# sony/timbre-trap

Measured on AMD Instinct MI355X. Metric: audio-seconds/s training throughput (9oct x 60bpo, 3s@22.05kHz), higher is better.
Workload: dtype bf16; 1 GPU; full train step (CQT x2 + AE fwd/bwd with consistency + 3 losses + clip + AdamW), model_complexity=2 latent=128, 64 clips x 3 s per GPU, under torch.autocast like reference experiments/train.py:415 (bf16 MFMA conv path of BASELINE config[2]; fp32 master weights, losses and optimizer); global_batch=64, parallelism=dp1

## Files before the change

include/ttrap.h:

```cpp
#ifndef TTRAP_H
#define TTRAP_H

#include <stdint.h>

#ifdef __cplusplus
extern "C" {
#endif

#define TT_E_BADARG      (-1)
#define TT_W_JOIN_LEFT 1
#define TT_E_UNSUPPORTED (-2)

#define TT_FLAG_BF16_OPERANDS 1
#define TT_FLAG_BF16_SPLIT    2

#define TT_ACT_NONE 0
#define TT_ACT_ELU  1
#define TT_ACT_RELU    2
#define TT_ACT_SIGMOID 3

int         tt_version(void);
const char* tt_arch(void);
const char* tt_error_string(int code);
int         tt_set_cu_limit(int cus);
// ... 124 lines not shown

int64_t tt_latent16_scratch_bytes(int B, int CT, int D, int E, int T);
int tt_latent16_contract(const void* in, const void* gy, const float* w, const float* bias, float* out, void* ws, int B, int CT,
                         int D, int Dout, int E, int T, void* stream);
int tt_latent16_expand(const float* z, int Dz, float fill, const float* w, const float* bias, void* out, void* ws, int B, int CT,
                       int D, int E, int T, void* stream);
int tt_latent16_pregated_ok(int CT, int D);
int tt_latent16_expand_gated(const float* z, const float* w, const void* gy, void* out, void* ws, int B, int CT, int D, int E, int T,
                             void* stream);
int tt_latent16_contract_pregated(const void* g, const float* w, float* out, void* ws, int B, int CT, int D, int Dout, int E, int T,
                                  void* stream);
int tt_latent16_wgrad_pregated(const float* z, int Dz, float fill, const void* g, float* dw, float* db, void* ws, int B, int CT, int D,
                               int E, int T, void* stream);
int tt_latent16_wgrad(const float* z, int Dz, float fill, const void* g, const void* gy, float* dw, float* db, void* ws, int B,
                      int CT, int D, int E, int T, void* stream);

int64_t tt_edge16_scratch_bytes(void);
int tt_convin16_fwd(const float* x, const float* w, const float* b, void* y, int B, int H, int T, void* stream);
int tt_convin16_bwd(const float* x, const void* y, const void* dy, const float* w, float* dx, float* dw, float* db, void* ws,
                    int B, int H, int T, void* stream);
int tt_convout16_fwd(const void* x, const float* w, const float* b, float* y, int B, int H, int T, void* stream);
int tt_convout16_bwd(const void* x, const float* dy, const float* w, void* dx, float* dw, float* db, void* ws, int B, int H,
                     int T, void* stream);
int tt_convin16_1_fwd(const float* x, const float* w, const float* b, void* y, int B, int H, int T, void* stream);
int tt_convin16_1_bwd(const float* x, const void* y, const void* dy, const float* w, float* dx, float* dw, float* db, void* ws, int B,
                      int H, int T, void* stream);
int tt_convout16_1_fwd(const void* x, const float* w, const float* b, float* y, int B, int H, int T, int act, void* stream);
int tt_convout16_1_bwd(const void* x, const float* y, const float* dy, const float* w, void* dx, float* dw, float* db, void* ws, int B,
                       int H, int T, int act, void* stream);

// ... 232 lines not shown
```

timbre-trap_amd/csrc/latent_bf16.hip:

```cpp
#include "bf16_common.h"

namespace {

#ifndef LAT_WGRAD_WAVES
#define LAT_WGRAD_WAVES 4
#endif
#ifndef LAT_EXPAND_Q
#define LAT_EXPAND_Q 2
#endif
#ifndef LAT_NSPLIT
#define LAT_NSPLIT 32
#endif

__device__ __forceinline__ float gate_f(float dy, float y) { return dy * elu_dout(y); }

template <int CT> __device__ __forceinline__ int ochc(int ct, int m) { return (CT / 4) * (m >> 2) + 4 * ct + (m & 3); }

template <int CT, int DT>
__global__ __launch_bounds__(NT) void k_lat_wprep1(const float* __restrict__ w, e16* __restrict__ wp, int D, int E) {
    constexpr int SPH = CT / 32;
    const int i = blockIdx.x * NT + threadIdx.x;
    if (i >= E * SPH * DT * 64) return;
    const int lane = i & 63, dt = (i >> 6) % DT, s = (i >> 6) / DT;
    const int h = s / SPH, half = s - h * SPH;
// ... 19 lines not shown
__global__ __launch_bounds__(NT) void k_lat_zprep(const float* __restrict__ z, e16* __restrict__ zt, int D, int Dz, float fill, int T,
                                                   long npix, float zscale, int one_row = -1) {
    constexpr int ZS = 32 * KS + 16, PCS = ZS / 8;
    const long i = (long)blockIdx.x * NT + threadIdx.x;
    const long pix = (i / (64 * PCS)) * 64 + (i & 63);
    if (pix >= npix) return;
    const int d0 = (int)((i >> 6) % PCS) * 8;
    const long b = pix / T, t = pix - b * T;
    e16x8 v;
#pragma unroll
    for (int e = 0; e < 8; ++e)
        v[e] = (e16)(zscale * (d0 + e < Dz ? z[(b * Dz + d0 + e) * T + t] : (d0 + e < D ? fill : (d0 + e == one_row ? 1.f : 0.f))));
    *reinterpret_cast<e16x8*>(zt + pix * ZS + d0) = v;
}

template <int CT, int DT, bool GATE, int QN>
__global__ __launch_bounds__(NT) void k_lat_contract(const e16* __restrict__ in, const e16* __restrict__ gy,
                                                      const e16* __restrict__ wp, const float* __restrict__ bias,
                                                      float* __restrict__ out, int D, int Dout, int E, int T, long npix, float oscale) {
    constexpr int SPH = CT / 32;
    constexpr int CHUNK = DT * 64 * 16, ROUNDS = (DT * 64 + NT - 1) / NT;
    extern __shared__ __align__(16) unsigned char smem[];
    const int tid = threadIdx.x, lane = tid & 63, wave = tid >> 6;
    const int n = lane & 15, g = lane >> 4;
    const int nsteps = E * SPH;
    const long p0 = (long)blockIdx.x * (64 * QN) + wave * (16 * QN);
    long pix[QN]; bool ok[QN]; long base[QN];
#pragma unroll
    for (int q = 0; q < QN; ++q) {
        pix[q] = p0 + 16 * q + n;
        ok[q] = pix[q] < npix;
        const long b = pix[q] / T, t = pix[q] - b * T;
        base[q] = (b * E * T + t) * CT + 8 * g;
    }
    auto stage = [&](int s, int buf) {
        const e16* src = wp + (long)s * (DT * 64 * 8);
#pragma unroll
        for (int r = 0; r < ROUNDS; ++r) {
            const int i = r * NT + wave * 64, p = i + lane;
            glds16(src + (long)(p < DT * 64 ? p : DT * 64 - 1) * 8, smem + buf * (ROUNDS * NT * 16) + (long)i * 16);
        }
    };
    auto fetch = [&](int s, e16x8 (&q8)[QN]) {
        const int h = s / SPH, half = s - h * SPH;
#pragma unroll
        for (int q = 0; q < QN; ++q) {
            const long off = base[q] + (long)h * T * CT + 32 * half;
            const bool live = ok[q] && s < nsteps;
            e16x8 v = *reinterpret_cast<const e16x8*>(in + (live ? off : 0));
            if (GATE) {
                const e16x8 yv = *reinterpret_cast<const e16x8*>(gy + (live ? off : 0));
#pragma unroll
                for (int e = 0; e < 8; ++e) v[e] = (e16)gate_f((float)v[e], (float)yv[e]);
            }
            if (!live)
#pragma unroll
                for (int e = 0; e < 8; ++e) v[e] = (e16)0.f;
            q8[q] = v;
        }
    };
    f32x4 acc[DT][QN];
#pragma unroll
    for (int dt = 0; dt < DT; ++dt)
#pragma unroll
        for (int q = 0; q < QN; ++q) acc[dt][q] = f32x4{0.f, 0.f, 0.f, 0.f};
    e16x8 bq[QN], bn[QN];
    stage(0, 0);
    fetch(0, bq);
    for (int s = 0; s < nsteps; ++s) {
        asm volatile("s_waitcnt vmcnt(0)" ::: "memory");
        __syncthreads();
        if (s + 1 < nsteps) stage(s + 1, (s + 1) & 1);
        fetch(s + 1, bn);
        const unsigned char* wb = smem + (s & 1) * (ROUNDS * NT * 16);
#pragma unroll
        for (int dt = 0; dt < DT; ++dt) {
            const e16x8 a = *reinterpret_cast<const e16x8*>(wb + ((long)dt * 64 + lane) * 16);
#pragma unroll
            for (int q = 0; q < QN; ++q) acc[dt][q] = mma32(a, bq[q], acc[dt][q]);
        }
#pragma unroll
        for (int q = 0; q < QN; ++q) bq[q] = bn[q];
    }
#pragma unroll
    for (int q = 0; q < QN; ++q) {
        if (!ok[q]) continue;
        const long b = pix[q] / T, t = pix[q] - b * T;
#pragma unroll
        for (int dt = 0; dt < DT; ++dt)
#pragma unroll
            for (int r = 0; r < 4; ++r) {
                const int d = 16 * dt + 4 * g + r;
                if (d < Dout) out[(b * Dout + d) * T + t] = acc[dt][q][r] * oscale + (bias ? bias[d] : 0.f);
            }
    }
    (void)CHUNK;
}

template <int CT, int KS, bool ACT, int QE, bool GOUT = false>
__global__ __launch_bounds__(NT) void k_lat_expand(const e16* __restrict__ zt, const e16* __restrict__ wp,
                                                    const float* __restrict__ bias, e16* __restrict__ out, int E, int T,
                                                    long npix, const e16* __restrict__ gy = nullptr) {
    constexpr int NC = CT / 16, NCH = CT / 4, ZS = 32 * KS + 16;
    constexpr int PCS = NC * KS * 64, ROUNDS = (PCS + NT - 1) / NT;
    extern __shared__ __align__(16) unsigned char smem[];
    const int tid = threadIdx.x, lane = tid & 63, wave = tid >> 6;
    const int n = lane & 15, g = lane >> 4;
    const long p0 = (long)blockIdx.x * (64 * QE) + wave * (16 * QE);
    e16x8 bz[QE][KS];
    long obase[QE]; bool ok[QE];
#pragma unroll
    for (int q = 0; q < QE; ++q) {
        const long pix = p0 + 16 * q + n;
        ok[q] = pix < npix;
        const long pc = ok[q] ? pix : 0;
#pragma unroll
        for (int s = 0; s < KS; ++s) bz[q][s] = *reinterpret_cast<const e16x8*>(zt + pc * ZS + 32 * s + 8 * g);
        const long b = pc / T, t = pc - b * T;
        obase[q] = (b * E * T + t) * CT + NCH * g;
    }
    float br[NCH];
#pragma unroll
    for (int e = 0; e < NCH; ++e) br[e] = ACT ? bias[NCH * g + e] : 0.f;
    auto stage = [&](int h, int buf) {
        const e16* src = wp + (long)h * (PCS * 8);
#pragma unroll
        for (int r = 0; r < ROUNDS; ++r) {
            const int i = r * NT + wave * 64, p = i + lane;
            glds16(src + (long)(p < PCS ? p : PCS - 1) * 8, smem + buf * (ROUNDS * NT * 16) + (long)i * 16);
        }
    };
    stage(0, 0);
    for (int h = 0; h < E; ++h) {
        asm volatile("s_waitcnt vmcnt(0)" ::: "memory");
        __syncthreads();
        if (h + 1 < E) stage(h + 1, (h + 1) & 1);
        const unsigned char* wb = smem + (h & 1) * (ROUNDS * NT * 16);
        f32x4 acc[NC][QE];
#pragma unroll
        for (int ct = 0; ct < NC; ++ct)
#pragma unroll
            for (int q = 0; q < QE; ++q) acc[ct][q] = f32x4{0.f, 0.f, 0.f, 0.f};
#pragma unroll
        for (int ct = 0; ct < NC; ++ct)
#pragma unroll
            for (int s = 0; s < KS; ++s) {
                const e16x8 a = *reinterpret_cast<const e16x8*>(wb + (((long)ct * KS + s) * 64 + lane) * 16);
#pragma unroll
                for (int q = 0; q < QE; ++q) acc[ct][q] = mma32(a, bz[q][s], acc[ct][q]);
            }
#pragma unroll
        for (int q = 0; q < QE; ++q) {
            if (!ok[q]) continue;
            e16* d = out + obase[q] + (long)h * T * CT;
#pragma unroll
            for (int c8 = 0; c8 < NCH / 8; ++c8) {
                e16x8 o, yv;
                if constexpr (GOUT) yv = *reinterpret_cast<const e16x8*>(gy + obase[q] + (long)h * T * CT + 8 * c8);
#pragma unroll
                for (int e = 0; e < 8; ++e) {
                    const int ch = 8 * c8 + e;
                    const float a = acc[ch >> 2][q][ch & 3] + br[ch];
                    o[e] = (e16)(ACT ? elu_f(a) : (GOUT ? a * elu_dout((float)yv[e]) : a));
                }
                *reinterpret_cast<e16x8*>(d + 8 * c8) = o;
            }
        }
    }
}

template <int CT> __device__ __forceinline__ int gswz(int p) { return CT == 64 ? ((p >> 1) & 3) : ((p >> 2) & 1); }

template <int CT, int DT, int KS, bool GATE>
__global__ __launch_bounds__(NT, LAT_WGRAD_WAVES) void k_lat_wgrad(const e16* __restrict__ zt, const e16* __restrict__ g_in,
                                                   const e16* __restrict__ gy, float* __restrict__ part,
                                                   float* __restrict__ dbpart, int E, int T, long npix, int nsplit) {
    constexpr int NC = CT / 16, ZS = 32 * KS + 16, ZB = ZS * 2, GB = CT * 2;
    constexpr int ZPC = 64 * ZB / 16, GPC = 64 * GB / 16;
    constexpr int ZR = (ZPC + NT - 1) / NT, GR = (GPC + NT - 1) / NT;
    constexpr int WPS = 4 / NC;
    extern __shared__ __align__(16) unsigned char smem[];
    unsigned char* zs = smem;
    unsigned char* gs = smem + ZR * NT * 16;
    const int tid = threadIdx.x, lane = tid & 63, wave = tid >> 6;
    const int n = lane & 15, g = lane >> 4, trj = n >> 2, trq = n & 3;
    const int h = blockIdx.x % E, ps = blockIdx.x / E;
    const int ct = wave % NC, sub0 = wave / NC;
    f32x4 acc[DT];
#pragma unroll
    for (int dt = 0; dt < DT; ++dt) acc[dt] = f32x4{0.f, 0.f, 0.f, 0.f};
    float dbacc[8] = {0.f, 0.f, 0.f, 0.f, 0.f, 0.f, 0.f, 0.f};
    const e16* zero = reinterpret_cast<const e16*>(&g_wzero16);
    const int npx = (int)npix, nchunks = (npx + 63) / 64;
    for (int ck = ps; ck < nchunks; ck += nsplit) {
        const int px0 = ck * 64;
        const int b0 = px0 / T, t00 = px0 - b0 * T;
        __syncthreads();
        const bool full = px0 + 64 <= npx;
        const e16* zc = zt + (long)px0 * ZS;
#pragma unroll
        for (int r = 0; r < ZR; ++r) {
            const int i = r * NT + wave * 64, p = i + lane;
            const bool okp = p < ZPC && (full || px0 + p * 16 / ZB < npx);
            glds16(okp ? zc + p * 8 : zero, zs + (long)i * 16);
        }
        e16x8 v[GATE ? GR : 1], yv[GATE ? GR : 1];
#pragma unroll
        for (int r = 0; r < GR; ++r) {
            const int i = r * NT + wave * 64, p = i + lane;
            const int q = p / (GB / 16), cgp = p % (GB / 16);
            const int cg = (((cgp >> 1) ^ gswz<CT>(q)) << 1) | (cgp & 1);
            const bool okp = p < GPC && (full || px0 + q < npx);
            int b = b0, t = t00 + q;
            if (T >= 64) { if (t >= T) { t -= T; ++b; } }
            else { const int e = t / T; b += e; t -= e * T; }
            const long off = okp ? (long)((b * E + h) * T + t) * CT + cg * 8 : 0;
            if constexpr (!GATE) glds16(okp ? g_in + off : zero, gs + (long)i * 16);
            else { v[r] = *reinterpret_cast<const e16x8*>(g_in + off); yv[r] = *reinterpret_cast<const e16x8*>(gy + off); }
        }
        if constexpr (GATE) {
#pragma unroll
            for (int r = 0; r < GR; ++r) {
                const int p = r * NT + tid;
                const bool okp = p < GPC && px0 + p / (GB / 16) < npx;
                e16x8 o;
#pragma unroll
                for (int e = 0; e < 8; ++e) {
                    const float gq = okp ? gate_f((float)v[r][e], (float)yv[r][e]) : 0.f;
                    dbacc[e] += gq;
                    o[e] = (e16)gq;
                }
                if (p < GPC) *reinterpret_cast<e16x8*>(gs + (long)p * 16) = o;
            }
        }
        asm volatile("s_waitcnt vmcnt(0)" ::: "memory");
        __syncthreads();
        for (int sub = sub0; sub < 2; sub += WPS) {
            s16x4 lo, hi;
            {
                const int p = 32 * sub + 4 * g + trj;
                lo = lds_tr16(gs + (long)p * GB + ((ct ^ gswz<CT>(p)) << 5) + 8 * trq);
                hi = lds_tr16(gs + (long)(p + 16) * GB + ((ct ^ gswz<CT>(p + 16)) << 5) + 8 * trq);
            }
            const e16x8 bq = __builtin_bit_cast(e16x8, __builtin_shufflevector(lo, hi, 0, 1, 2, 3, 4, 5, 6, 7));
#pragma unroll
            for (int dt = 0; dt < DT; ++dt) {
                const int p = 32 * sub + 4 * g + trj;
                const s16x4 alo = lds_tr16(zs + (long)p * ZB + dt * 32 + 8 * trq);
                const s16x4 ahi = lds_tr16(zs + (long)(p + 16) * ZB + dt * 32 + 8 * trq);
                acc[dt] = mma32(__builtin_bit_cast(e16x8, __builtin_shufflevector(alo, ahi, 0, 1, 2, 3, 4, 5, 6, 7)), bq, acc[dt]);
            }
        }
    }
    float* pw = part + ((long)blockIdx.x * 4 + wave) * (DT * 256);
#pragma unroll
    for (int dt = 0; dt < DT; ++dt)
#pragma unroll
        for (int r = 0; r < 4; ++r) pw[(dt * 4 + r) * 64 + lane] = acc[dt][r];
    if constexpr (GATE) {
        __syncthreads();
        float* dl = reinterpret_cast<float*>(smem);
#pragma unroll
        for (int e = 0; e < 8; ++e) dl[tid * 8 + e] = dbacc[e];
        __syncthreads();
        if (tid < CT) {
            float sum = 0.f;
            for (int t2 = 0; t2 < NT; ++t2) {
                const int q = t2 / (GB / 16), cgp = t2 % (GB / 16);
                const int cg = (((cgp >> 1) ^ gswz<CT>(q)) << 1) | (cgp & 1);
                if (cg == (tid >> 3)) sum += dl[t2 * 8 + (tid & 7)];
            }
            dbpart[(long)blockIdx.x * 64 + tid] = sum;
        }
// ... 31 lines not shown
    float t = 0.f;
    for (int h = 0; h < E; ++h) t += rows[h * CT + c];
    db[c] += t;
}

constexpr int NSPLIT = LAT_NSPLIT;

template <int CT, int DT, int KS> struct LatSizes {
    static constexpr int SPH = CT / 32, NC = CT / 16, ZS = 32 * KS + 16;
    static long wp1_bytes(int E) { return (long)E * SPH * DT * 64 * 16; }
    static long wp2_bytes(int E) { return (long)E * NC * KS * 64 * 16; }
    static long zt_bytes(long npix) { return npix * ZS * 2 + 4096; }
    static long part_bytes(int E) { return ((long)NSPLIT * E * 4 * DT * 256 + (long)NSPLIT * E * 64) * 4; }
};

template <int CT, int DT, int KS, bool GATE>
int run_contract(const e16* in, const e16* gy, const float* w, const float* bias, float* out, unsigned char* ws, int B, int D,
                 int Dout, int E, int T, hipStream_t st, bool pregated = false) {
    using L = LatSizes<CT, DT, KS>;
    const long npix = (long)B * T;
    e16* wp = reinterpret_cast<e16*>(ws);
    const int pieces = E * L::SPH * DT * 64;
    hipLaunchKernelGGL((k_lat_wprep1<CT, DT>), dim3((pieces + NT - 1) / NT), dim3(NT), 0, st, w, wp, D, E);
    TT_LAUNCH_CHECK();
    constexpr int ROUNDS = (DT * 64 + NT - 1) / NT, LDS = 2 * ROUNDS * NT * 16;
    static AttrOnce once;
#ifndef TT_LAT_QN64
#define TT_LAT_QN64 1
#endif
    constexpr int QN = CT == 64 ? TT_LAT_QN64 : 4;
    auto kern = k_lat_contract<CT, DT, GATE, QN>;
    if (int rc = raise_lds(kern, LDS, once)) return rc;
    const float oscale = (GATE || pregated) ? tt_loss_unscale() : 1.f;
    hipLaunchKernelGGL(kern, dim3((unsigned)((npix + 64 * QN - 1) / (64 * QN))), dim3(NT), LDS, st, in, gy, wp, bias, out, D, Dout, E, T, npix, oscale);
    TT_LAUNCH_CHECK();
    return 0;
}

template <int CT, int DT, int KS, bool ACT, bool GOUT = false>
int run_expand(const float* z, int Dz, float fill, const float* w, const float* bias, e16* out, unsigned char* ws, int B, int D, int E,
               int T, hipStream_t st, const e16* gy = nullptr) {
    using L = LatSizes<CT, DT, KS>;
    const long npix = (long)B * T;
    e16* wp = reinterpret_cast<e16*>(ws);
    e16* zt = reinterpret_cast<e16*>(ws + ((L::wp2_bytes(E) + 255) / 256) * 256);
    const int pieces = E * L::NC * KS * 64;
    hipLaunchKernelGGL((k_lat_wprep2<CT, KS>), dim3((pieces + NT - 1) / NT), dim3(NT), 0, st, w, wp, D, E);
    TT_LAUNCH_CHECK();
    const long zp = ((npix + 63) / 64) * 64 * (L::ZS / 8);
    hipLaunchKernelGGL((k_lat_zprep<KS>), dim3((unsigned)((zp + NT - 1) / NT)), dim3(NT), 0, st, z, zt, D, Dz, fill, T, npix,
                       ACT ? 1.f : tt_loss_scale());
    TT_LAUNCH_CHECK();
    constexpr int PCS = L::NC * KS * 64, ROUNDS = (PCS + NT - 1) / NT, LDS = 2 * ROUNDS * NT * 16;
    static AttrOnce once;
    constexpr int QE = LAT_EXPAND_Q;
    auto kern = k_lat_expand<CT, KS, ACT, QE, GOUT>;
    if (int rc = raise_lds(kern, LDS, once)) return rc;
    hipLaunchKernelGGL(kern, dim3((unsigned)((npix + 64 * QE - 1) / (64 * QE))), dim3(NT), LDS, st, zt, wp, bias, out, E, T, npix, gy);
    TT_LAUNCH_CHECK();
    return 0;
}

template <int CT, int DT, int KS, bool GATE>
int run_wgrad(const float* z, int Dz, float fill, const e16* g_in, const e16* gy, float* dw, float* db, unsigned char* ws, int B,
              int D, int E, int T, hipStream_t st, bool pregated = false) {
    using L = LatSizes<CT, DT, KS>;
    const long npix = (long)B * T;
    if (npix >= (1l << 30) || (long)B * E * T >= (1l << 31)) return TT_E_UNSUPPORTED;
    e16* zt = reinterpret_cast<e16*>(ws);
    float* part = reinterpret_cast<float*>(ws + ((L::zt_bytes(npix) + 255) / 256) * 256);
    float* dbpart = part + (long)NSPLIT * E * 4 * DT * 256;
    const long zp = ((npix + 63) / 64) * 64 * (L::ZS / 8);
    if (pregated && (GATE || D >= 16 * DT || !db)) return TT_E_UNSUPPORTED;
    const int one_row = pregated ? D : -1;
    hipLaunchKernelGGL((k_lat_zprep<KS>), dim3((unsigned)((zp + NT - 1) / NT)), dim3(NT), 0, st, z, zt, D, Dz, fill, T, npix,
                       (GATE || pregated) ? 1.f : tt_loss_scale(), one_row);
    TT_LAUNCH_CHECK();
    constexpr int ZB = L::ZS * 2, GBY = CT * 2;
    constexpr int ZR = (64 * ZB / 16 + NT - 1) / NT, GR = (64 * GBY / 16 + NT - 1) / NT;
    constexpr int LDS0 = (ZR + GR) * NT * 16, LDS = LDS0 > NT * 32 ? LDS0 : NT * 32;
    static AttrOnce once;
    auto kern = k_lat_wgrad<CT, DT, KS, GATE>;
    if (int rc = raise_lds(kern, LDS, once)) return rc;
    hipLaunchKernelGGL(kern, dim3(E * NSPLIT), dim3(NT), LDS, st, zt, g_in, gy, part, dbpart, E, T, npix, NSPLIT);
    TT_LAUNCH_CHECK();
    const int total = E * (CT / 16) * DT * 256 + CT * 16;
    hipLaunchKernelGGL((k_lat_wred<CT, DT>), dim3((total + NT - 1) / NT), dim3(NT), 0, st, part, dbpart, dw, (GATE || pregated) ? db : nullptr, D, E,
                       NSPLIT, tt_loss_unscale(), one_row, dbpart);
    TT_LAUNCH_CHECK();
    if (pregated) {
        static_assert(CT <= 64, "one wave sums the channels");
        hipLaunchKernelGGL(k_lat_dbrows, dim3(1), dim3(64), 0, st, dbpart, db, E, CT);
        TT_LAUNCH_CHECK();
    }
    return 0;
}

inline int cfg_of(int CT, int D) {
    if (CT == 32 && D >= 1 && D <= 48) return 1;
    if (CT == 64 && D >= 1 && D <= 144) return 2;
    return 0;
}

}

extern "C" {

int64_t tt_latent16_scratch_bytes(int B, int CT, int D, int E, int T) {
    const long npix = (long)B * T;
    switch (cfg_of(CT, D)) {
        case 1: { using L = LatSizes<32, 3, 2>; return L::wp1_bytes(E) + L::wp2_bytes(E) + L::zt_bytes(npix) + L::part_bytes(E) + 4096; }
        case 2: { using L = LatSizes<64, 9, 5>; return L::wp1_bytes(E) + L::wp2_bytes(E) + L::zt_bytes(npix) + L::part_bytes(E) + 4096; }
    }
    return -1;
}

int tt_latent16_contract(const void* in, const void* gy, const float* w, const float* bias, float* out, void* ws, int B, int CT, int D,
                         int Dout, int E, int T, void* stream) {
    if (!in || !w || !out || !ws || B <= 0 || E <= 0 || T <= 0 || T % 16 || Dout < 1 || Dout > D) return TT_E_BADARG;
// ... 79 lines not shown
```

timbre-trap_amd/csrc/losses.hip:

```cpp
#include "common.h"

namespace {

constexpr int MAXP = 1024;

__device__ __forceinline__ void block_partial(double v, double* partials) {
    __shared__ double red[4];
    v = wave_sum_d(v);
    if ((threadIdx.x & 63) == 0) red[threadIdx.x >> 6] = v;
    __syncthreads();
    if (threadIdx.x == 0) partials[blockIdx.x] = red[0] + red[1] + red[2] + red[3];
}

__global__ __launch_bounds__(256) void k_finalize(const double* __restrict__ partials, int n, double scale,
                                                  float* __restrict__ out, int take_sqrt) {
    __shared__ double red[4];
    double v = 0.0;
    for (int i = threadIdx.x; i < n; i += 256) v += partials[i];
    v = wave_sum_d(v);
    if ((threadIdx.x & 63) == 0) red[threadIdx.x >> 6] = v;
    __syncthreads();
    if (threadIdx.x == 0) {
        double s = (red[0] + red[1] + red[2] + red[3]) * scale;
        out[0] = (float)(take_sqrt ? sqrt(s) : s);
// ... 625 lines not shown

thread_local float g_tt_loss_scale = 1.0f;
extern "C" float tt_set_loss_scale(float scale) {
    const float prev = g_tt_loss_scale;
    if (scale > 0.f && scale <= 16777216.f) g_tt_loss_scale = scale;
    return prev;
}

int g_tt_cu_limit = 256;
extern "C" int tt_set_cu_limit(int cus) {
    const int prev = g_tt_cu_limit;
    if (cus > 0) g_tt_cu_limit = cus > 256 ? 256 : cus;
    return prev;
}

extern "C" int tt_version(void) { return 13; }
extern "C" const char* tt_arch(void) { return "gfx950"; }
extern "C" const char* tt_error_string(int code) {
    if (code == 0) return "ok";
    if (code == TT_E_BADARG) return "ttrap: bad argument";
    if (code == TT_E_UNSUPPORTED) return "ttrap: unsupported shape or option";
    return hipGetErrorString((hipError_t)code);
}
```

timbre-trap_amd/timbre_trap/_hip.py:

```python

import ctypes
import os
import subprocess
import sys

_HERE = os.path.dirname(os.path.abspath(__file__))
PKG_ROOT = os.path.dirname(_HERE)
REPO_ROOT = os.path.dirname(PKG_ROOT)
CSRC = os.path.join(PKG_ROOT, 'csrc')
LIB_PATH = os.path.join(PKG_ROOT, 'lib', 'libttrap_hip.so')
if os.environ.get('TTRAP_LIB'):
    LIB_PATH = os.path.join(PKG_ROOT, 'lib', os.environ['TTRAP_LIB'])
SOURCES = ['cqt.hip', 'cqt_generic.hip', 'conv_generic.hip', 'conv_mfma.hip', 'conv_small.hip', 'conv_wide_bf16.hip', 'conv_level_bf16.hip', 'conv_stride_bf16.hip',
           'latent_bf16.hip', 'conv_edge_bf16.hip', 'gemm.hip', 'losses.hip', 'magnitude.hip',
           'conv_wide_f16.hip', 'conv_level_f16.hip', 'conv_stride_f16.hip', 'latent_f16.hip', 'conv_edge_f16.hip',
           'conv_x3.hip',
           'sdr.hip',
           'mpe.hip',
           'resample.hip',
           'notes.hip']

_lib = None

c_void_p, c_int, c_int64, c_float = ctypes.c_void_p, ctypes.c_int, ctypes.c_int64, ctypes.c_float
# ... 76 lines not shown
    'tt_sconv16_fwd': (c_int, [P, P, P, P, I, I, I, I, P]),
    'tt_sconv16_bwd': (c_int, [P, P, P, P, P, P, P, P, I, I, I, I, P]),
    'tt_tconv16_fwd': (c_int, [P, P, P, P, I, I, I, I, I, P]),
    'tt_tconv16_bwd': (c_int, [P, P, P, P, P, P, P, P, I, I, I, I, I, P]),
    'tt_gate16': (c_int, [P, P, L, P]),
    'tt_sconv16_bwd_pregated': (c_int, [P, P, P, P, P, P, P, I, I, I, I, P]),
    'tt_tconv16_bwd_pregated': (c_int, [P, P, P, P, P, P, P, I, I, I, I, I, I, P]),
    'tt_latent16_pregated_ok': (c_int, [I, I]),
    'tt_latent16_expand_gated': (c_int, [P, P, P, P, P, I, I, I, I, I, P]),
    'tt_latent16_contract_pregated': (c_int, [P, P, P, P, I, I, I, I, I, I, P]),
    'tt_latent16_wgrad_pregated': (c_int, [P, I, F_, P, P, P, P, I, I, I, I, I, P]),
    'tt_latent16_scratch_bytes': (c_int64, [I, I, I, I, I]),
    'tt_latent16_contract': (c_int, [P, P, P, P, P, P, I, I, I, I, I, I, P]),
    'tt_latent16_expand': (c_int, [P, I, F_, P, P, P, P, I, I, I, I, I, P]),
    'tt_latent16_wgrad': (c_int, [P, I, F_, P, P, P, P, P, I, I, I, I, I, P]),
    'tt_edge16_scratch_bytes': (c_int64, []),
    'tt_convin16_fwd': (c_int, [P, P, P, P, I, I, I, P]),
    'tt_convin16_bwd': (c_int, [P, P, P, P, P, P, P, P, I, I, I, P]),
    'tt_convout16_fwd': (c_int, [P, P, P, P, I, I, I, P]),
    'tt_convout16_bwd': (c_int, [P, P, P, P, P, P, P, I, I, I, P]),
    'tt_convin16_1_fwd': (c_int, [P, P, P, P, I, I, I, P]),
    'tt_convin16_1_bwd': (c_int, [P, P, P, P, P, P, P, P, I, I, I, P]),
    'tt_convout16_1_fwd': (c_int, [P, P, P, P, I, I, I, I, P]),
    'tt_convout16_1_bwd': (c_int, [P, P, P, P, P, P, P, P, I, I, I, I, P]),
    'tt_sconv_fwd': (c_int, [P, P, P, P, I, I, I, I, P]),
    'tt_wgrad_scratch_floats': (c_int64, []),
    'tt_sconv_bwd': (c_int, [P, P, P, P, P, P, P, P, I, I, I, I, P]),
    'tt_tconv_fwd': (c_int, [P, P, P, P, I, I, I, I, I, P]),
    'tt_tconv_bwd': (c_int, [P, P, P, P, P, P, P, P, I, I, I, I, I, P]),
    'tt_gemm': (c_int, [P, P, P, P, I, I, I, I, I, L, L, L, I, L, L, L, I, F_, F_, I, I, I, P]),
# ... 173 lines not shown
```

Measured before the change: 3881 audio-seconds/s.

## Restage latent contract/expand/wgrad kernels over multiple rows per LDS stage

Restructures the latent bottleneck kernels. The contract kernel now stages several K-steps of weights per barrier (KSTG). The expand kernel stages two rows of weights per stage (RS=2) and uses four pixel groups per wave on large inputs. The weight-gradient kernel processes several frequency rows per workgroup (HB), with optional double-buffered or two-chunk staging and an XCD-grouped block order. The aim is fewer barriers and fewer redundant z-tile loads, at the cost of more LDS and registers per workgroup and so possibly lower occupancy. A runtime geometry setter is added to tune the variants.

Result: no change. 3880 audio-seconds/s (-0.0%).

```diff
diff --git a/include/ttrap.h b/include/ttrap.h
--- a/include/ttrap.h
+++ b/include/ttrap.h
@@ -162,6 +162,7 @@
                                int E, int T, void* stream);
 int tt_latent16_wgrad(const float* z, int Dz, float fill, const void* g, const void* gy, float* dw, float* db, void* ws, int B,
                       int CT, int D, int E, int T, void* stream);
+int tt_latent16_set_geometry(int kstg, int hb);
 
 int64_t tt_edge16_scratch_bytes(void);
 int tt_convin16_fwd(const float* x, const float* w, const float* b, void* y, int B, int H, int T, void* stream);
diff --git a/timbre-trap_amd/csrc/latent_bf16.hip b/timbre-trap_amd/csrc/latent_bf16.hip
--- a/timbre-trap_amd/csrc/latent_bf16.hip
+++ b/timbre-trap_amd/csrc/latent_bf16.hip
@@ -1,4 +1,10 @@
 #include "bf16_common.h"
+
+#ifndef TT_F16
+int g_tt_lat_kstg = 0, g_tt_lat_hb = 0;
+#else
+extern int g_tt_lat_kstg, g_tt_lat_hb;
+#endif
 
 namespace {
 
@@ -57,16 +63,17 @@
     *reinterpret_cast<e16x8*>(zt + pix * ZS + d0) = v;
 }
 
-template <int CT, int DT, bool GATE, int QN>
+template <int CT, int DT, bool GATE, int QN, int KSTG>
 __global__ __launch_bounds__(NT) void k_lat_contract(const e16* __restrict__ in, const e16* __restrict__ gy,
                                                       const e16* __restrict__ wp, const float* __restrict__ bias,
                                                       float* __restrict__ out, int D, int Dout, int E, int T, long npix, float oscale) {
     constexpr int SPH = CT / 32;
-    constexpr int CHUNK = DT * 64 * 16, ROUNDS = (DT * 64 + NT - 1) / NT;
+    constexpr int SPC = KSTG * DT * 64, ROUNDS = (SPC + NT - 1) / NT;
     extern __shared__ __align__(16) unsigned char smem[];
     const int tid = threadIdx.x, lane = tid & 63, wave = tid >> 6;
     const int n = lane & 15, g = lane >> 4;
-    const int nsteps = E * SPH;
+    const int nsteps = E * SPH, nstages = (nsteps + KSTG - 1) / KSTG;
+    const int wpieces = nsteps * DT * 64;
     const long p0 = (long)blockIdx.x * (64 * QN) + wave * (16 * QN);
     long pix[QN]; bool ok[QN]; long base[QN];
 #pragma unroll
@@ -76,30 +83,34 @@
         const long b = pix[q] / T, t = pix[q] - b * T;
         base[q] = (b * E * T + t) * CT + 8 * g;
     }
-    auto stage = [&](int s, int buf) {
-        const e16* src = wp + (long)s * (DT * 64 * 8);
+    auto stage = [&](int sg, int buf) {
+        const int first = sg * SPC;
 #pragma unroll
         for (int r = 0; r < ROUNDS; ++r) {
-            const int i = r * NT + wave * 64, p = i + lane;
-            glds16(src + (long)(p < DT * 64 ? p : DT * 64 - 1) * 8, smem + buf * (ROUNDS * NT * 16) + (long)i * 16);
+            const int i = r * NT + wave * 64, p = first + i + lane;
+            glds16(wp + (long)(p < wpieces ? p : wpieces - 1) * 8, smem + buf * (ROUNDS * NT * 16) + (long)i * 16);
         }
     };
-    auto fetch = [&](int s, e16x8 (&q8)[QN]) {
-        const int h = s / SPH, half = s - h * SPH;
-#pragma unroll
-        for (int q = 0; q < QN; ++q) {
-            const long off = base[q] + (long)h * T * CT + 32 * half;
-            const bool live = ok[q] && s < nsteps;
-            e16x8 v = *reinterpret_cast<const e16x8*>(in + (live ? off : 0));
-            if (GATE) {
-                const e16x8 yv = *reinterpret_cast<const e16x8*>(gy + (live ? off : 0));
-#pragma unroll
-                for (int e = 0; e < 8; ++e) v[e] = (e16)gate_f((float)v[e], (float)yv[e]);
-            }
-            if (!live)
-#pragma unroll
-                for (int e = 0; e < 8; ++e) v[e] = (e16)0.f;
-            q8[q] = v;
+    auto fetch = [&](int sg, e16x8 (&q8)[KSTG][QN]) {
+#pragma unroll
+        for (int k = 0; k < KSTG; ++k) {
+            const int s = sg * KSTG + k;
+            const int h = s / SPH, half = s - h * SPH;
+#pragma unroll
+            for (int q = 0; q < QN; ++q) {
+                const long off = base[q] + (long)h * T * CT + 32 * half;
+                const bool live = ok[q] && s < nsteps;
+                e16x8 v = *reinterpret_cast<const e16x8*>(in + (live ? off : 0));
+                if (GATE) {
+                    const e16x8 yv = *reinterpret_cast<const e16x8*>(gy + (live ? off : 0));
+#pragma unroll
+                    for (int e = 0; e < 8; ++e) v[e] = (e16)gate_f((float)v[e], (float)yv[e]);
+                }
+                if (!live)
+#pragma unroll
+                    for (int e = 0; e < 8; ++e) v[e] = (e16)0.f;
+                q8[k][q] = v;
+            }
         }
     };
     f32x4 acc[DT][QN];
@@ -107,23 +118,30 @@
     for (int dt = 0; dt < DT; ++dt)
 #pragma unroll
         for (int q = 0; q < QN; ++q) acc[dt][q] = f32x4{0.f, 0.f, 0.f, 0.f};
-    e16x8 bq[QN], bn[QN];
+    e16x8 bq[KSTG][QN], bn[KSTG][QN];
     stage(0, 0);
     fetch(0, bq);
-    for (int s = 0; s < nsteps; ++s) {
+    for (int sg = 0; sg < nstages; ++sg) {
         asm volatile("s_waitcnt vmcnt(0)" ::: "memory");
         __syncthreads();
-        if (s + 1 < nsteps) stage(s + 1, (s + 1) & 1);
-        fetch(s + 1, bn);
-        const unsigned char* wb = smem + (s & 1) * (ROUNDS * NT * 16);
-#pragma unroll
-        for (int dt = 0; dt < DT; ++dt) {
-            const e16x8 a = *reinterpret_cast<const e16x8*>(wb + ((long)dt * 64 + lane) * 16);
-#pragma unroll
-            for (int q = 0; q < QN; ++q) acc[dt][q] = mma32(a, bq[q], acc[dt][q]);
-        }
-#pragma unroll
-        for (int q = 0; q < QN; ++q) bq[q] = bn[q];
+        if (sg + 1 < nstages) stage(sg + 1, (sg + 1) & 1);
+        fetch(sg + 1, bn);
+        const unsigned char* wb = smem + (sg & 1) * (ROUNDS * NT * 16);
+#pragma unroll
+        for (int k = 0; k < KSTG; ++k) {
+            if (sg * KSTG + k < nsteps) {
+#pragma unroll
+                for (int dt = 0; dt < DT; ++dt) {
+                    const e16x8 a = *reinterpret_cast<const e16x8*>(wb + (((long)k * DT + dt) * 64 + lane) * 16);
+#pragma unroll
+                    for (int q = 0; q < QN; ++q) acc[dt][q] = mma32(a, bq[k][q], acc[dt][q]);
+                }
+            }
+        }
+#pragma unroll
+        for (int k = 0; k < KSTG; ++k)
+#pragma unroll
+            for (int q = 0; q < QN; ++q) bq[k][q] = bn[k][q];
     }
 #pragma unroll
     for (int q = 0; q < QN; ++q) {
@@ -137,19 +155,19 @@
                 if (d < Dout) out[(b * Dout + d) * T + t] = acc[dt][q][r] * oscale + (bias ? bias[d] : 0.f);
             }
     }
-    (void)CHUNK;
-}
-
-template <int CT, int KS, bool ACT, int QE, bool GOUT = false>
+}
+
+template <int CT, int KS, bool ACT, int QE, bool GOUT = false, int RS = 1>
 __global__ __launch_bounds__(NT) void k_lat_expand(const e16* __restrict__ zt, const e16* __restrict__ wp,
                                                     const float* __restrict__ bias, e16* __restrict__ out, int E, int T,
                                                     long npix, const e16* __restrict__ gy = nullptr) {
     constexpr int NC = CT / 16, NCH = CT / 4, ZS = 32 * KS + 16;
-    constexpr int PCS = NC * KS * 64, ROUNDS = (PCS + NT - 1) / NT;
+    constexpr int PCS = NC * KS * 64, SPC = RS * PCS, ROUNDS = (SPC + NT - 1) / NT;
     extern __shared__ __align__(16) unsigned char smem[];
     const int tid = threadIdx.x, lane = tid & 63, wave = tid >> 6;
     const int n = lane & 15, g = lane >> 4;
     const long p0 = (long)blockIdx.x * (64 * QE) + wave * (16 * QE);
+    const int nstages = (E + RS - 1) / RS, wpieces = E * PCS;
     e16x8 bz[QE][KS];
     long obase[QE]; bool ok[QE];
 #pragma unroll
@@ -165,48 +183,53 @@
     float br[NCH];
 #pragma unroll
     for (int e = 0; e < NCH; ++e) br[e] = ACT ? bias[NCH * g + e] : 0.f;
-    auto stage = [&](int h, int buf) {
-        const e16* src = wp + (long)h * (PCS * 8);
+    auto stage = [&](int sg, int buf) {
+        const int first = sg * SPC;
 #pragma unroll
         for (int r = 0; r < ROUNDS; ++r) {
-            const int i = r * NT + wave * 64, p = i + lane;
-            glds16(src + (long)(p < PCS ? p : PCS - 1) * 8, smem + buf * (ROUNDS * NT * 16) + (long)i * 16);
+            const int i = r * NT + wave * 64, p = first + i + lane;
+            glds16(wp + (long)(p < wpieces ? p : wpieces - 1) * 8, smem + buf * (ROUNDS * NT * 16) + (long)i * 16);
         }
     };
     stage(0, 0);
-    for (int h = 0; h < E; ++h) {
+    for (int sg = 0; sg < nstages; ++sg) {
         asm volatile("s_waitcnt vmcnt(0)" ::: "memory");
         __syncthreads();
-        if (h + 1 < E) stage(h + 1, (h + 1) & 1);
-        const unsigned char* wb = smem + (h & 1) * (ROUNDS * NT * 16);
-        f32x4 acc[NC][QE];
-#pragma unroll
-        for (int ct = 0; ct < NC; ++ct)
-#pragma unroll
-            for (int q = 0; q < QE; ++q) acc[ct][q] = f32x4{0.f, 0.f, 0.f, 0.f};
-#pragma unroll
-        for (int ct = 0; ct < NC; ++ct)
-#pragma unroll
-            for (int s = 0; s < KS; ++s) {
-                const e16x8 a = *reinterpret_cast<const e16x8*>(wb + (((long)ct * KS + s) * 64 + lane) * 16);
-#pragma unroll
-                for (int q = 0; q < QE; ++q) acc[ct][q] = mma32(a, bz[q][s], acc[ct][q]);
-            }
-#pragma unroll
-        for (int q = 0; q < QE; ++q) {
-            if (!ok[q]) continue;
-            e16* d = out + obase[q] + (long)h * T * CT;
-#pragma unroll
-            for (int c8 = 0; c8 < NCH / 8; ++c8) {
-                e16x8 o, yv;
-                if constexpr (GOUT) yv = *reinterpret_cast<const e16x8*>(gy + obase[q] + (long)h * T * CT + 8 * c8);
-#pragma unroll
-                for (int e = 0; e < 8; ++e) {
-                    const int ch = 8 * c8 + e;
-                    const float a = acc[ch >> 2][q][ch & 3] + br[ch];
-                    o[e] = (e16)(ACT ? elu_f(a) : (GOUT ? a * elu_dout((float)yv[e]) : a));
+        if (sg + 1 < nstages) stage(sg + 1, (sg + 1) & 1);
+#pragma unroll
+        for (int k = 0; k < RS; ++k) {
+            const int h = sg * RS + k;
+            if (h >= E) break;
+            const unsigned char* wb = smem + (sg & 1) * (ROUNDS * NT * 16) + (long)k * PCS * 16;
+            f32x4 acc[NC][QE];
+#pragma unroll
+            for (int ct = 0; ct < NC; ++ct)
+#pragma unroll
+                for (int q = 0; q < QE; ++q) acc[ct][q] = f32x4{0.f, 0.f, 0.f, 0.f};
+#pragma unroll
+            for (int ct = 0; ct < NC; ++ct)
+#pragma unroll
+                for (int s = 0; s < KS; ++s) {
+                    const e16x8 a = *reinterpret_cast<const e16x8*>(wb + (((long)ct * KS + s) * 64 + lane) * 16);
+#pragma unroll
+                    for (int q = 0; q < QE; ++q) acc[ct][q] = mma32(a, bz[q][s], acc[ct][q]);
                 }
-                *reinterpret_cast<e16x8*>(d + 8 * c8) = o;
+#pragma unroll
+            for (int q = 0; q < QE; ++q) {
+                if (!ok[q]) continue;
+                e16* d = out + obase[q] + (long)h * T * CT;
+#pragma unroll
+                for (int c8 = 0; c8 < NCH / 8; ++c8) {
+                    e16x8 o, yv;
+                    if constexpr (GOUT) yv = *reinterpret_cast<const e16x8*>(gy + obase[q] + (long)h * T * CT + 8 * c8);
+#pragma unroll
+                    for (int e = 0; e < 8; ++e) {
+                        const int ch = 8 * c8 + e;
+                        const float a = acc[ch >> 2][q][ch & 3] + br[ch];
+                        o[e] = (e16)(ACT ? elu_f(a) : (GOUT ? a * elu_dout((float)yv[e]) : a));
+                    }
+                    *reinterpret_cast<e16x8*>(d + 8 * c8) = o;
+                }
             }
         }
     }
@@ -214,31 +237,40 @@
 
 template <int CT> __device__ __forceinline__ int gswz(int p) { return CT == 64 ? ((p >> 1) & 3) : ((p >> 2) & 1); }
 
-template <int CT, int DT, int KS, bool GATE>
-__global__ __launch_bounds__(NT, LAT_WGRAD_WAVES) void k_lat_wgrad(const e16* __restrict__ zt, const e16* __restrict__ g_in,
+template <int CT, int DT, int KS, bool GATE, int HB = 1, bool DBUF = false, bool XG = false, int CKS = 1>
+__global__ __launch_bounds__(NT, HB == 1 ? LAT_WGRAD_WAVES : 2) void k_lat_wgrad(const e16* __restrict__ zt, const e16* __restrict__ g_in,
                                                    const e16* __restrict__ gy, float* __restrict__ part,
                                                    float* __restrict__ dbpart, int E, int T, long npix, int nsplit) {
+    static_assert(!GATE || (HB == 1 && !DBUF && !XG && CKS == 1), "the gated form stages through registers: one row, one chunk, one buffer, dumps by workgroup");
     constexpr int NC = CT / 16, ZS = 32 * KS + 16, ZB = ZS * 2, GB = CT * 2;
     constexpr int ZPC = 64 * ZB / 16, GPC = 64 * GB / 16;
     constexpr int ZR = (ZPC + NT - 1) / NT, GR = (GPC + NT - 1) / NT;
+    constexpr int SUBB = (ZR + HB * GR) * NT * 16, BUFB = CKS * SUBB;
     constexpr int WPS = 4 / NC;
     extern __shared__ __align__(16) unsigned char smem[];
-    unsigned char* zs = smem;
-    unsigned char* gs = smem + ZR * NT * 16;
     const int tid = threadIdx.x, lane = tid & 63, wave = tid >> 6;
     const int n = lane & 15, g = lane >> 4, trj = n >> 2, trq = n & 3;
-    const int h = blockIdx.x % E, ps = blockIdx.x / E;
+    const int nhb = (E + HB - 1) / HB;
+    int hg = blockIdx.x % nhb, ps = blockIdx.x / nhb;
+    if constexpr (XG) {
+        const int idx = blockIdx.x >> 3;
+        hg = idx % nhb;
+        ps = (blockIdx.x & 7) + 8 * (idx / nhb);
+    }
+    const int h0 = hg * HB;
+    const int nh = E - h0 < HB ? E - h0 : HB;
     const int ct = wave % NC, sub0 = wave / NC;
-    f32x4 acc[DT];
-#pragma unroll
-    for (int dt = 0; dt < DT; ++dt) acc[dt] = f32x4{0.f, 0.f, 0.f, 0.f};
+    f32x4 acc[HB][DT];
+#pragma unroll
+    for (int j = 0; j < HB; ++j)
+#pragma unroll
+        for (int dt = 0; dt < DT; ++dt) acc[j][dt] = f32x4{0.f, 0.f, 0.f, 0.f};
     float dbacc[8] = {0.f, 0.f, 0.f, 0.f, 0.f, 0.f, 0.f, 0.f};
     const e16* zero = reinterpret_cast<const e16*>(&g_wzero16);
     const int npx = (int)npix, nchunks = (npx + 63) / 64;
-    for (int ck = ps; ck < nchunks; ck += nsplit) {
+    auto stage1 = [&](int ck, unsigned char* zs) {
         const int px0 = ck * 64;
         const int b0 = px0 / T, t00 = px0 - b0 * T;
-        __syncthreads();
         const bool full = px0 + 64 <= npx;
         const e16* zc = zt + (long)px0 * ZS;
 #pragma unroll
@@ -249,57 +281,101 @@
         }
         e16x8 v[GATE ? GR : 1], yv[GATE ? GR : 1];
 #pragma unroll
-        for (int r = 0; r < GR; ++r) {
-            const int i = r * NT + wave * 64, p = i + lane;
-            const int q = p / (GB / 16), cgp = p % (GB / 16);
-            const int cg = (((cgp >> 1) ^ gswz<CT>(q)) << 1) | (cgp & 1);
-            const bool okp = p < GPC && (full || px0 + q < npx);
-            int b = b0, t = t00 + q;
-            if (T >= 64) { if (t >= T) { t -= T; ++b; } }
-            else { const int e = t / T; b += e; t -= e * T; }
-            const long off = okp ? (long)((b * E + h) * T + t) * CT + cg * 8 : 0;
-            if constexpr (!GATE) glds16(okp ? g_in + off : zero, gs + (long)i * 16);
-            else { v[r] = *reinterpret_cast<const e16x8*>(g_in + off); yv[r] = *reinterpret_cast<const e16x8*>(gy + off); }
-        }
-        if constexpr (GATE) {
+        for (int j = 0; j < HB; ++j) {
+            if (j >= nh) break;
+            unsigned char* gs = zs + (ZR + j * GR) * NT * 16;
+            const int h = h0 + j;
 #pragma unroll
             for (int r = 0; r < GR; ++r) {
-                const int p = r * NT + tid;
-                const bool okp = p < GPC && px0 + p / (GB / 16) < npx;
-                e16x8 o;
-#pragma unroll
-                for (int e = 0; e < 8; ++e) {
-                    const float gq = okp ? gate_f((float)v[r][e], (float)yv[r][e]) : 0.f;
-                    dbacc[e] += gq;
-                    o[e] = (e16)gq;
+                const int i = r * NT + wave * 64, p = i + lane;
+                const int q = p / (GB / 16), cgp = p % (GB / 16);
+                const int cg = (((cgp >> 1) ^ gswz<CT>(q)) << 1) | (cgp & 1);
+                const bool okp = p < GPC && (full || px0 + q < npx);
+                int b = b0, t = t00 + q;
+                if (T >= 64) { if (t >= T) { t -= T; ++b; } }
+                else { const int e = t / T; b += e; t -= e * T; }
+                const long off = okp ? (long)((b * E + h) * T + t) * CT + cg * 8 : 0;
+                if constexpr (!GATE) glds16(okp ? g_in + off : zero, gs + (long)i * 16);
+                else { v[r] = *reinterpret_cast<const e16x8*>(g_in + off); yv[r] = *reinterpret_cast<const e16x8*>(gy + off); }
+            }
+            if constexpr (GATE) {
+#pragma unroll
+                for (int r = 0; r < GR; ++r) {
+                    const int p = r * NT + tid;
+                    const bool okp = p < GPC && px0 + p / (GB / 16) < npx;
+                    e16x8 o;
+#pragma unroll
+                    for (int e = 0; e < 8; ++e) {
+                        const float gq = okp ? gate_f((float)v[r][e], (float)yv[r][e]) : 0.f;
+                        dbacc[e] += gq;
+                        o[e] = (e16)gq;
+                    }
+                    if (p < GPC) *reinterpret_cast<e16x8*>(gs + (long)p * 16) = o;
                 }
-                if (p < GPC) *reinterpret_cast<e16x8*>(gs + (long)p * 16) = o;
-            }
-        }
-        asm volatile("s_waitcnt vmcnt(0)" ::: "memory");
-        __syncthreads();
+            }
+        }
+    };
+    auto stage = [&](int ck, int buf) {
+#pragma unroll
+        for (int c = 0; c < CKS; ++c)
+            if (ck + c * nsplit < nchunks) stage1(ck + c * nsplit, smem + buf * BUFB + c * SUBB);
+    };
+    auto compute1 = [&](const unsigned char* zs) {
         for (int sub = sub0; sub < 2; sub += WPS) {
-            s16x4 lo, hi;
-            {
-                const int p = 32 * sub + 4 * g + trj;
-                lo = lds_tr16(gs + (long)p * GB + ((ct ^ gswz<CT>(p)) << 5) + 8 * trq);
-                hi = lds_tr16(gs + (long)(p + 16) * GB + ((ct ^ gswz<CT>(p + 16)) << 5) + 8 * trq);
-            }
-            const e16x8 bq = __builtin_bit_cast(e16x8, __builtin_shufflevector(lo, hi, 0, 1, 2, 3, 4, 5, 6, 7));
+            const int p = 32 * sub + 4 * g + trj;
+            e16x8 bq[HB];
+#pragma unroll
+            for (int j = 0; j < HB; ++j) {
+                if (j >= nh) break;
+                const unsigned char* gs = zs + (ZR + j * GR) * NT * 16;
+                const s16x4 lo = lds_tr16(gs + (long)p * GB + ((ct ^ gswz<CT>(p)) << 5) + 8 * trq);
+                const s16x4 hi = lds_tr16(gs + (long)(p + 16) * GB + ((ct ^ gswz<CT>(p + 16)) << 5) + 8 * trq);
+                bq[j] = __builtin_bit_cast(e16x8, __builtin_shufflevector(lo, hi, 0, 1, 2, 3, 4, 5, 6, 7));
+            }
 #pragma unroll
             for (int dt = 0; dt < DT; ++dt) {
-                const int p = 32 * sub + 4 * g + trj;
                 const s16x4 alo = lds_tr16(zs + (long)p * ZB + dt * 32 + 8 * trq);
                 const s16x4 ahi = lds_tr16(zs + (long)(p + 16) * ZB + dt * 32 + 8 * trq);
-                acc[dt] = mma32(__builtin_bit_cast(e16x8, __builtin_shufflevector(alo, ahi, 0, 1, 2, 3, 4, 5, 6, 7)), bq, acc[dt]);
-            }
-        }
-    }
-    float* pw = part + ((long)blockIdx.x * 4 + wave) * (DT * 256);
-#pragma unroll
-    for (int dt = 0; dt < DT; ++dt)
-#pragma unroll
-        for (int r = 0; r < 4; ++r) pw[(dt * 4 + r) * 64 + lane] = acc[dt][r];
+                const e16x8 a = __builtin_bit_cast(e16x8, __builtin_shufflevector(alo, ahi, 0, 1, 2, 3, 4, 5, 6, 7));
+#pragma unroll
+                for (int j = 0; j < HB; ++j)
+                    if (j < nh) acc[j][dt] = mma32(a, bq[j], acc[j][dt]);
+            }
+        }
+    };
+    auto compute = [&](int ck, int buf) {
+#pragma unroll
+        for (int c = 0; c < CKS; ++c)
+            if (ck + c * nsplit < nchunks) compute1(smem + buf * BUFB + c * SUBB);
+    };
+    const int step = CKS * nsplit;
+    if constexpr (DBUF) {
+        if (ps < nchunks) stage(ps, 0);
+        int buf = 0;
+        for (int ck = ps; ck < nchunks; ck += step, buf ^= 1) {
+            asm volatile("s_waitcnt vmcnt(0)" ::: "memory");
+            __syncthreads();
+            if (ck + step < nchunks) stage(ck + step, buf ^ 1);
+            compute(ck, buf);
+        }
+    } else {
+        for (int ck = ps; ck < nchunks; ck += step) {
+            __syncthreads();
+            stage(ck, 0);
+            asm volatile("s_waitcnt vmcnt(0)" ::: "memory");
+            __syncthreads();
+            compute(ck, 0);
+        }
+    }
+#pragma unroll
+    for (int j = 0; j < HB; ++j) {
+        if (j >= nh) break;
+        float* pw = part + (((long)ps * E + h0 + j) * 4 + wave) * (DT * 256);
+#pragma unroll
+        for (int dt = 0; dt < DT; ++dt)
+#pragma unroll
+            for (int r = 0; r < 4; ++r) pw[(dt * 4 + r) * 64 + lane] = acc[j][dt][r];
+    }
     if constexpr (GATE) {
         __syncthreads();
         float* dl = reinterpret_cast<float*>(smem);
@@ -361,6 +437,42 @@
     static long part_bytes(int E) { return ((long)NSPLIT * E * 4 * DT * 256 + (long)NSPLIT * E * 64) * 4; }
 };
 
+#ifndef TT_LAT_QN64
+#define TT_LAT_QN64 1
+#endif
+
+template <int CT, int DT, bool GATE, int QN, int KSTG>
+int launch_contract(const e16* in, const e16* gy, const e16* wp, const float* bias, float* out, int D, int Dout, int E, int T, long npix,
+                    float oscale, hipStream_t st) {
+    constexpr int ROUNDS = (KSTG * DT * 64 + NT - 1) / NT, LDS = 2 * ROUNDS * NT * 16;
+    static AttrOnce once;
+    auto kern = k_lat_contract<CT, DT, GATE, QN, KSTG>;
+    if (int rc = raise_lds(kern, LDS, once)) return rc;
+    hipLaunchKernelGGL(kern, dim3((unsigned)((npix + 64 * QN - 1) / (64 * QN))), dim3(NT), LDS, st, in, gy, wp, bias, out, D, Dout, E, T, npix, oscale);
+    TT_LAUNCH_CHECK();
+    return 0;
+}
+
+#ifndef TT_LAT_DEFAULT_KSTG
+#define TT_LAT_DEFAULT_KSTG 4
+#endif
+#ifndef TT_LAT_DEFAULT_QN
+#define TT_LAT_DEFAULT_QN 2
+#endif
+inline void contract_geometry(int CT, long npix, int& kstg, int& qn) {
+    const int knob = g_tt_lat_kstg;
+    kstg = knob & 15;
+    qn = knob >> 4;
+    if (CT != 64) {
+        if (!kstg) kstg = 1;
+        qn = 4;
+        return;
+    }
+    if (kstg == 1 && !qn) qn = TT_LAT_QN64;
+    if (!kstg) kstg = TT_LAT_DEFAULT_KSTG;
+    if (!qn) qn = (TT_LAT_DEFAULT_QN == 2 && npix >= 2l * 128 * tt_cus()) ? 2 : 1;
+}
+
 template <int CT, int DT, int KS, bool GATE>
 int run_contract(const e16* in, const e16* gy, const float* w, const float* bias, float* out, unsigned char* ws, int B, int D,
                  int Dout, int E, int T, hipStream_t st, bool pregated = false) {
@@ -370,16 +482,35 @@
     const int pieces = E * L::SPH * DT * 64;
     hipLaunchKernelGGL((k_lat_wprep1<CT, DT>), dim3((pieces + NT - 1) / NT), dim3(NT), 0, st, w, wp, D, E);
     TT_LAUNCH_CHECK();
-    constexpr int ROUNDS = (DT * 64 + NT - 1) / NT, LDS = 2 * ROUNDS * NT * 16;
+    const float oscale = (GATE || pregated) ? tt_loss_unscale() : 1.f;
+    int kstg, qn;
+    contract_geometry(CT, npix, kstg, qn);
+#define TT_LAT_CONTRACT(QN_, KSTG_) return launch_contract<CT, DT, GATE, QN_, KSTG_>(in, gy, wp, bias, out, D, Dout, E, T, npix, oscale, st)
+    if constexpr (CT == 64) {
+        if (qn == 1) { if (kstg == 1) TT_LAT_CONTRACT(1, 1); if (kstg == 2) TT_LAT_CONTRACT(1, 2); if (kstg == 4) TT_LAT_CONTRACT(1, 4); }
+        if (qn == 2) { if (kstg == 1) TT_LAT_CONTRACT(2, 1); if (kstg == 2) TT_LAT_CONTRACT(2, 2); if (kstg == 4) TT_LAT_CONTRACT(2, 4); }
+    } else {
+        if (kstg == 1) TT_LAT_CONTRACT(4, 1); if (kstg == 2) TT_LAT_CONTRACT(4, 2); if (kstg == 4) TT_LAT_CONTRACT(4, 4);
+    }
+#undef TT_LAT_CONTRACT
+    return TT_E_UNSUPPORTED;
+}
+
+#ifndef TT_LAT_DEFAULT_EXPAND_RS
+#define TT_LAT_DEFAULT_EXPAND_RS 2
+#endif
+#ifndef TT_LAT_DEFAULT_EXPAND_Q4
+#define TT_LAT_DEFAULT_EXPAND_Q4 1
+#endif
+static_assert(LAT_EXPAND_Q == 2, "k_lat_expand's launcher dispatches 2 or 4 groups per wave");
+
+template <int CT, int KS, bool ACT, int QE, bool GOUT, int RS>
+int launch_expand(const e16* zt, const e16* wp, const float* bias, e16* out, int E, int T, long npix, const e16* gy, hipStream_t st) {
+    constexpr int SPC = RS * (CT / 16) * KS * 64, ROUNDS = (SPC + NT - 1) / NT, LDS = 2 * ROUNDS * NT * 16;
     static AttrOnce once;
-#ifndef TT_LAT_QN64
-#define TT_LAT_QN64 1
-#endif
-    constexpr int QN = CT == 64 ? TT_LAT_QN64 : 4;
-    auto kern = k_lat_contract<CT, DT, GATE, QN>;
+    auto kern = k_lat_expand<CT, KS, ACT, QE, GOUT, RS>;
     if (int rc = raise_lds(kern, LDS, once)) return rc;
-    const float oscale = (GATE || pregated) ? tt_loss_unscale() : 1.f;
-    hipLaunchKernelGGL(kern, dim3((unsigned)((npix + 64 * QN - 1) / (64 * QN))), dim3(NT), LDS, st, in, gy, wp, bias, out, D, Dout, E, T, npix, oscale);
+    hipLaunchKernelGGL(kern, dim3((unsigned)((npix + 64 * QE - 1) / (64 * QE))), dim3(NT), LDS, st, zt, wp, bias, out, E, T, npix, gy);
     TT_LAUNCH_CHECK();
     return 0;
 }
@@ -398,12 +529,33 @@
     hipLaunchKernelGGL((k_lat_zprep<KS>), dim3((unsigned)((zp + NT - 1) / NT)), dim3(NT), 0, st, z, zt, D, Dz, fill, T, npix,
                        ACT ? 1.f : tt_loss_scale());
     TT_LAUNCH_CHECK();
-    constexpr int PCS = L::NC * KS * 64, ROUNDS = (PCS + NT - 1) / NT, LDS = 2 * ROUNDS * NT * 16;
+    const int knob = g_tt_lat_kstg;
+    int rs = (knob & 15) ? ((knob & 15) >= 2 ? 2 : 1) : 0, qe = 2 * (knob >> 4);
+    if ((knob & 15) == 1 && !qe) qe = LAT_EXPAND_Q;
+    if (!rs) rs = CT == 64 ? TT_LAT_DEFAULT_EXPAND_RS : 1;
+    if (!qe) qe = (CT == 64 && TT_LAT_DEFAULT_EXPAND_Q4 && npix >= 2l * 256 * tt_cus()) ? 4 : LAT_EXPAND_Q;
+#define TT_LAT_EXPAND(QE_, RS_) return launch_expand<CT, KS, ACT, QE_, GOUT, RS_>(zt, wp, bias, out, E, T, npix, gy, st)
+    if (qe == 2) { if (rs == 1) TT_LAT_EXPAND(2, 1); else TT_LAT_EXPAND(2, 2); }
+    if (qe == 4) { if (rs == 1) TT_LAT_EXPAND(4, 1); else TT_LAT_EXPAND(4, 2); }
+#undef TT_LAT_EXPAND
+    return TT_E_UNSUPPORTED;
+}
+
+#ifndef TT_LAT_DEFAULT_HB
+#define TT_LAT_DEFAULT_HB (2 + 64)
+#endif
+
+template <int CT, int DT, int KS, bool GATE, int HB, bool DBUF, bool XG = false, int CKS = 1>
+int launch_wgrad(const e16* zt, const e16* g_in, const e16* gy, float* part, float* dbpart, int E, int T, long npix, hipStream_t st) {
+    constexpr int ZB = (32 * KS + 16) * 2, GBY = CT * 2;
+    constexpr int ZR = (64 * ZB / 16 + NT - 1) / NT, GR = (64 * GBY / 16 + NT - 1) / NT;
+    constexpr int LDS0 = (DBUF ? 2 : 1) * CKS * (ZR + HB * GR) * NT * 16, LDS = LDS0 > NT * 32 ? LDS0 : NT * 32;
+    static_assert(LDS <= 160 * 1024, "staging buffers beyond the LDS of a CU");
     static AttrOnce once;
-    constexpr int QE = LAT_EXPAND_Q;
-    auto kern = k_lat_expand<CT, KS, ACT, QE, GOUT>;
+    static_assert(!XG || NSPLIT % 8 == 0, "the XCD-grouped order deals whole splits to the 8 XCDs");
+    auto kern = k_lat_wgrad<CT, DT, KS, GATE, HB, DBUF, XG, CKS>;
     if (int rc = raise_lds(kern, LDS, once)) return rc;
-    hipLaunchKernelGGL(kern, dim3((unsigned)((npix + 64 * QE - 1) / (64 * QE))), dim3(NT), LDS, st, zt, wp, bias, out, E, T, npix, gy);
+    hipLaunchKernelGGL(kern, dim3(((E + HB - 1) / HB) * NSPLIT), dim3(NT), LDS, st, zt, g_in, gy, part, dbpart, E, T, npix, NSPLIT);
     TT_LAUNCH_CHECK();
     return 0;
 }
@@ -423,14 +575,24 @@
     hipLaunchKernelGGL((k_lat_zprep<KS>), dim3((unsigned)((zp + NT - 1) / NT)), dim3(NT), 0, st, z, zt, D, Dz, fill, T, npix,
                        (GATE || pregated) ? 1.f : tt_loss_scale(), one_row);
     TT_LAUNCH_CHECK();
-    constexpr int ZB = L::ZS * 2, GBY = CT * 2;
-    constexpr int ZR = (64 * ZB / 16 + NT - 1) / NT, GR = (64 * GBY / 16 + NT - 1) / NT;
-    constexpr int LDS0 = (ZR + GR) * NT * 16, LDS = LDS0 > NT * 32 ? LDS0 : NT * 32;
-    static AttrOnce once;
-    auto kern = k_lat_wgrad<CT, DT, KS, GATE>;
-    if (int rc = raise_lds(kern, LDS, once)) return rc;
-    hipLaunchKernelGGL(kern, dim3(E * NSPLIT), dim3(NT), LDS, st, zt, g_in, gy, part, dbpart, E, T, npix, NSPLIT);
-    TT_LAUNCH_CHECK();
+    int knob = g_tt_lat_hb;
+    if (!(knob & 15)) knob = CT == 64 ? TT_LAT_DEFAULT_HB : 1;
+    const int hb = GATE ? 1 : (knob & 15);
+    const bool cks2 = hb > 1 && (knob & 64), dbuf = hb > 1 && !(knob & 16) && !cks2, xg = !GATE && (knob & 32);
+    int rc = TT_E_UNSUPPORTED;
+#define TT_LAT_WGRAD(HB_, DB_, XG_) rc = launch_wgrad<CT, DT, KS, false, HB_, DB_, XG_>(zt, g_in, gy, part, dbpart, E, T, npix, st)
+    if constexpr (!GATE) {
+        if (hb == 1) { if (xg) TT_LAT_WGRAD(1, false, true); else TT_LAT_WGRAD(1, false, false); }
+        if (cks2 && hb == 2) rc = launch_wgrad<CT, DT, KS, false, 2, false, false, 2>(zt, g_in, gy, part, dbpart, E, T, npix, st);
+        else if (cks2 && hb == 4) rc = launch_wgrad<CT, DT, KS, false, 4, false, false, 2>(zt, g_in, gy, part, dbpart, E, T, npix, st);
+        else if (hb == 2) { if (xg) { if (dbuf) TT_LAT_WGRAD(2, true, true); else TT_LAT_WGRAD(2, false, true); }
+                       else { if (dbuf) TT_LAT_WGRAD(2, true, false); else TT_LAT_WGRAD(2, false, false); } }
+        else if (hb == 4) { if (dbuf) TT_LAT_WGRAD(4, true, false); else TT_LAT_WGRAD(4, false, false); }
+    } else {
+        rc = launch_wgrad<CT, DT, KS, true, 1, false>(zt, g_in, gy, part, dbpart, E, T, npix, st);
+    }
+#undef TT_LAT_WGRAD
+    if (rc) return rc;
     const int total = E * (CT / 16) * DT * 256 + CT * 16;
     hipLaunchKernelGGL((k_lat_wred<CT, DT>), dim3((total + NT - 1) / NT), dim3(NT), 0, st, part, dbpart, dw, (GATE || pregated) ? db : nullptr, D, E,
                        NSPLIT, tt_loss_unscale(), one_row, dbpart);
@@ -450,6 +612,17 @@
 }
 
 }
+
+#ifndef TT_F16
+extern "C" int tt_latent16_set_geometry(int kstg, int hb) {
+    const int ks = kstg & 15, qn = kstg >> 4, h = hb & 15;
+    if (kstg < 0 || hb < 0 || (ks != 0 && ks != 1 && ks != 2 && ks != 4) || qn > 2 || (h != 0 && h != 1 && h != 2 && h != 4) || (hb >> 7) || (h == 4 && (hb & 32)) || ((hb & 64) && (h < 2 || (hb & 32))) || (h == 0 && hb != 0) || (ks == 0 && kstg != 0))
+        return TT_E_BADARG;
+    g_tt_lat_kstg = kstg;
+    g_tt_lat_hb = hb;
+    return 0;
+}
+#endif
 
 extern "C" {
 
diff --git a/timbre-trap_amd/csrc/losses.hip b/timbre-trap_amd/csrc/losses.hip
--- a/timbre-trap_amd/csrc/losses.hip
+++ b/timbre-trap_amd/csrc/losses.hip
@@ -663,7 +663,7 @@
     return prev;
 }
 
-extern "C" int tt_version(void) { return 13; }
+extern "C" int tt_version(void) { return 14; }
 extern "C" const char* tt_arch(void) { return "gfx950"; }
 extern "C" const char* tt_error_string(int code) {
     if (code == 0) return "ok";
diff --git a/timbre-trap_amd/timbre_trap/_hip.py b/timbre-trap_amd/timbre_trap/_hip.py
--- a/timbre-trap_amd/timbre_trap/_hip.py
+++ b/timbre-trap_amd/timbre_trap/_hip.py
@@ -114,6 +114,7 @@
     'tt_latent16_contract': (c_int, [P, P, P, P, P, P, I, I, I, I, I, I, P]),
     'tt_latent16_expand': (c_int, [P, I, F_, P, P, P, P, I, I, I, I, I, P]),
     'tt_latent16_wgrad': (c_int, [P, I, F_, P, P, P, P, P, I, I, I, I, I, P]),
+    'tt_latent16_set_geometry': (c_int, [I, I]),
     'tt_edge16_scratch_bytes': (c_int64, []),
     'tt_convin16_fwd': (c_int, [P, P, P, P, I, I, I, P]),
     'tt_convin16_bwd': (c_int, [P, P, P, P, P, P, P, P, I, I, I, P]),
```
